# jczarnowski/DeepFactors

Hardware: NVIDIA H100
Metric: keyframe-pair Jacobian+JtJ evals/sec (640x480, C=32) (higher is better)
Workload: dtype f32

## Files before the change

### deepfactors_b200/csrc/dfk_api.cu

```cuda
#include <cuda_runtime.h>
#include <math.h>
#include <stdint.h>
#include <stdio.h>
#include <stdlib.h>
#include <string.h>

#include <algorithm>
#include <cmath>
#include <memory>
#include <new>
#include <string>
#include <vector>

#include "dfk.h"
#include "dfk_internal.h"

using namespace dfk;

namespace {

template <typename T, bool Pinned>
struct Scratch {
  T* ptr = nullptr;
  size_t cap = 0;

  Scratch() = default;
  Scratch(Scratch&& o) noexcept : ptr(o.ptr), cap(o.cap) { o.ptr = nullptr; o.cap = 0; }
  ~Scratch() { release(); }

  void release()
  {
    if constexpr (Pinned) cudaFreeHost(ptr);
    else cudaFree(ptr);
    ptr = nullptr;
    cap = 0;
  }
  cudaError_t ensure(size_t need)
  {
    if (cap >= need) return cudaSuccess;
    const size_t n = std::max(need, cap * 2);
    release();
    void* p = nullptr;
    const cudaError_t e = Pinned ? cudaMallocHost(&p, n * sizeof(T)) : cudaMalloc(&p, n * sizeof(T));
    if (e != cudaSuccess) return e;
    ptr = static_cast<T*>(p);
    cap = n;
    return e;
  }
};
template <typename T>
using DeviceBuf = Scratch<T, false>;
template <typename T>
using PinnedBuf = Scratch<T, true>;

}

struct DfkContext {
  int device = 0;
  int num_sms = 1;
  int sm_limit = 0;
  cudaStream_t own_stream = nullptr;
  cudaStream_t stream = nullptr;
  std::string err;
  DfkSfmAlignerParams params;
  DfkGramMode gram_mode = DFK_GRAM_AUTO;
  float se3_huber_delta = 0.1f;

  DeviceBuf<float> simple_scratch;
  DeviceBuf<unsigned int> counter;
  DeviceBuf<float> out_dev;
  PinnedBuf<float> out_host;
  DeviceBuf<float> code_dev;
  DeviceBuf<float> track_dev;
  PinnedBuf<float> track_host;
  DeviceBuf<unsigned char> batch_dev;
  PinnedBuf<unsigned char> batch_host;
  DeviceBuf<float> batch_partials;
  DeviceBuf<unsigned int> batch_counters;

  DeviceBuf<unsigned char> sparse_dev;
  PinnedBuf<unsigned char> sparse_host;
  DeviceBuf<unsigned char> rep_dev;
  std::vector<unsigned char> rep_host;
  DeviceBuf<unsigned char> geo_dev;
  std::vector<unsigned char> geo_host;
  DeviceBuf<SfmItemDev> items_dev;
  DeviceBuf<float> partials_dev;
  DeviceBuf<int> window_lists;
  DeviceBuf<int> marg_lists;
  DeviceBuf<double> marg_code;
  DeviceBuf<double> marg_dev;
  struct RayTab {
    float fx, fy, u0, v0;
    uint32_t w, h;
    DeviceBuf<float> dev;
    bool built;
  };
  std::vector<RayTab> ray_cache;
  std::vector<size_t> ray_pending;
  bool ray_flush = false;
  DeviceBuf<float> codes_dev;
  std::vector<float> codes_host;
  DeviceBuf<float> records_dev;
  PinnedBuf<float> records_host;
  std::vector<SfmItemDev> items_host;

  bool profiling = false;
  std::vector<cudaEvent_t> ev_pool;
  size_t ev_used = 0;
  double ev_ms_accum = 0.0;
  uint64_t ev_count_accum = 0;
  uint64_t launches = 0;

  ~DfkContext()
  {
    for (cudaEvent_t e : ev_pool) cudaEventDestroy(e);
    if (own_stream) cudaStreamDestroy(own_stream);
  }
};

struct DfkSfmStream {
  int device = 0, code_size = 0, max_items = 0, depth = 0;
  size_t max_bytes = 0;
  cudaStream_t copy_stream = nullptr;
  struct Slot {
    DeviceBuf<unsigned char> dev;
    DeviceBuf<float> rec_dev;
    PinnedBuf<float> rec_host;
    cudaEvent_t uploaded = nullptr, done = nullptr;
    int n = 0;
    uint64_t ticket = 0;
    bool busy = false;
  };
  std::vector<Slot> slots;
  std::vector<DfkSfmWorkItem> dev_items;
  uint64_t next_ticket = 0, next_wait = 0;
};

struct DfkWindow {
  int device = 0;
  WindowDev dev{};
  DeviceBuf<int> ints;
  DeviceBuf<float> areas;
  size_t floats = 0;
  std::vector<int> pair_k0, pair_k1, link_k0, link_k1, item_pair;
  std::vector<int> prior_ptr{0}, prior_kf, blk_i, blk_j;
  std::vector<long long> prior_off;
  DeviceBuf<int> kp_ints;
  DeviceBuf<long long> kp_off;
  KfPriorDev kp{};
};

struct DfkWindowSolver {
  int device = 0;
  int num_vars = 0, code_size = 0, num_keyframes = 0;
  WindowSolverDev* dev = nullptr;
  ~DfkWindowSolver() { window_solver_destroy(dev); }
};

namespace {

DfkStatus fail(DfkHandle h, DfkStatus s, const std::string& msg)
{
  if (h) h->err = msg;
  return s;
}

DfkStatus oom(DfkHandle h) noexcept
{
  if (h) {
    try {
      h->err = "out of host memory";
    } catch (...) {
    }
  }
  return DFK_ERR_NOMEM;
}

template <class F>
DfkStatus guarded(DfkHandle h, F&& body) noexcept
{
  if (!h) return DFK_ERR_INVALID_ARG;
  try {
    return body();
  } catch (...) {
    return oom(h);
  }
}
// ... 277 lines not shown
    if (fused) d.flags |= ITEM_FLAG_FUSED_DEPTH;
  }
  const int T = (int)tile_cursor;
  int G = std::min(max_ctas, T);
  if (G < 1) G = 1;
  plan->num_items = n;
  plan->num_tiles = T;
  plan->num_ctas = G;
  uint32_t partial_cursor = 0;
  int c = 0;
  for (int i = 0; i < n; ++i) {
    SfmItemDev& d = h->items_host[i];
    const long long tb = d.tile_begin, te = tb + d.num_tiles;
    while ((long long)(c + 1) * T / G <= tb) ++c;
    int first = c, last = c;
    while ((long long)(last + 1) * T / G < te) ++last;
    d.first_cta = (uint32_t)first;
    d.num_ctas = (uint32_t)(last - first + 1);
    d.partial_begin = partial_cursor;
    partial_cursor += d.num_ctas;
  }
  plan->num_partials = (int)partial_cursor;
  return DFK_OK;
}

constexpr size_t kMaxEventPairs = 8192;

DfkStatus drain_events(DfkHandle h)
{
  if (h->ev_used == 0) return DFK_OK;
  DFK_CUDA(h, cudaStreamSynchronize(h->stream), "profiling: stream synchronize failed");
  for (size_t k = 0; k < h->ev_used; ++k) {
    float ms = 0.f;
    DFK_CUDA(h, cudaEventElapsedTime(&ms, h->ev_pool[2 * k], h->ev_pool[2 * k + 1]), "profiling: event read failed");
    h->ev_ms_accum += ms;
  }
  h->ev_count_accum += h->ev_used;
  h->ev_used = 0;
  return DFK_OK;
}

DfkStatus profile_events(DfkHandle h, cudaEvent_t* e0, cudaEvent_t* e1)
{
  if (h->ev_used == kMaxEventPairs) DFK_TRY(drain_events(h));
  while (h->ev_pool.size() < 2 * (h->ev_used + 1)) {
    cudaEvent_t e;
    DFK_CUDA(h, cudaEventCreate(&e), "profiling: event creation failed");
    h->ev_pool.push_back(e);
  }
  *e0 = h->ev_pool[2 * h->ev_used];
  *e1 = h->ev_pool[2 * h->ev_used + 1];
  h->ev_used += 1;
  return DFK_OK;
}

DfkStatus run_batch(DfkHandle h, const DfkSfmWorkItem* items, int n, int code_size, float* records_dev)
{
  if (!items || n <= 0 || !records_dev) return fail(h, DFK_ERR_INVALID_ARG, "[SfmAligner::RunStep] null/empty batch");
  const bool wide = sfm_wide_supported(code_size);
  if (!sfm_fp32_supported(code_size) && !wide)
    return fail(h, DFK_ERR_UNSUPPORTED,
                "[SfmAligner::RunStep] no kernel instantiated for code size " + std::to_string(code_size));
  const bool tc_ok = sfm_tc_supported(code_size) || sfm_tc_wide_supported(code_size);
  bool tc = (h->gram_mode == DFK_GRAM_TF32X3) || (h->gram_mode == DFK_GRAM_AUTO && tc_ok);
  if (tc) {
    bool grads_ok = true;
    for (int i = 0; i < n && grads_ok; ++i)
      grads_ok = items[i].grad1.ptr && aligned(items[i].grad1.ptr, 8) && (items[i].grad1.pitch_bytes % 8 == 0);
    if (!grads_ok) {
      if (h->gram_mode == DFK_GRAM_TF32X3)
        return fail(h, DFK_ERR_UNSUPPORTED, "[SfmAligner::RunStep] tensor-core path needs 8-byte aligned grad1 rows");
      tc = false;
    }
  }
  if (tc && !tc_ok)
    return fail(h, DFK_ERR_UNSUPPORTED,
                "[SfmAligner::RunStep] tensor-core Gram path is not instantiated for code size " +
                    std::to_string(code_size));
  DeviceGuard guard(h->device);
  SfmLaunchPlan plan;
  const int tile_px = tc ? sfm_tc_tile_pixels(code_size) : (wide ? sfm_wide_tile_pixels(code_size) : kTilePixels);
  bool any_fused = false;
  for (int i = 0; i < n; ++i) any_fused = any_fused || items[i].code != nullptr;
  if (any_fused) {
    DFK_CUDA(h, h->codes_dev.ensure((size_t)n * code_size), "[SfmAligner::RunStep] scratch allocation failed");
    h->codes_host.assign((size_t)n * code_size, 0.0f);
  }
  const int ctas_per_sm = tc ? sfm_tc_ctas_per_sm(code_size) : (wide ? 1 : sfm_fp32_ctas_per_sm(code_size));
  const int sms = (h->sm_limit > 0 && h->sm_limit < h->num_sms) ? h->sm_limit : h->num_sms;
  DFK_TRY(build_items(h, items, n, code_size, tile_px, ctas_per_sm * sms, h->codes_dev.ptr, &plan));
  if (any_fused)
    DFK_CUDA(h, cudaMemcpyAsync(h->codes_dev.ptr, h->codes_host.data(), sizeof(float) * (size_t)n * code_size,
                                cudaMemcpyHostToDevice, h->stream),
             "[SfmAligner::RunStep] code upload failed");
  const size_t pfloats = tc ? sfm_tc_partial_floats(code_size) : sfm_partial_floats(code_size);
  DFK_CUDA(h, h->items_dev.ensure((size_t)n), "[SfmAligner::RunStep] scratch allocation failed");
  DFK_CUDA(h, h->partials_dev.ensure((size_t)plan.num_partials * pfloats), "[SfmAligner::RunStep] scratch allocation failed");
  SfmItemDev* items_dev = h->items_dev.ptr;
  float* partials_dev = h->partials_dev.ptr;
  DFK_CUDA(h, cudaMemcpyAsync(items_dev, h->items_host.data(), sizeof(SfmItemDev) * n, cudaMemcpyHostToDevice, h->stream),
           "[SfmAligner::RunStep] work list upload failed");
  if (!h->ray_pending.empty()) {
    DFK_CUDA(h, launch_sfm_ray_tables(items_dev, n, h->stream), "[SfmAligner::RunStep] kernel launch failed");
    for (size_t rt : h->ray_pending) h->ray_cache[rt].built = true;
    h->launches += 1;
  }
  cudaEvent_t ev0 = nullptr, ev1 = nullptr;
  if (h->profiling) DFK_TRY(profile_events(h, &ev0, &ev1));
  if (tc && wide) {
    DFK_CUDA(h, launch_sfm_tc_wide(code_size, items_dev, plan, partials_dev, h->stream, ev0, ev1),
             "[SfmAligner::RunStep] kernel launch failed");
  } else if (tc) {
    DFK_CUDA(h, launch_sfm_tc(items_dev, plan, partials_dev, h->stream, ev0, ev1),
             "[SfmAligner::RunStep] kernel launch failed");
  } else if (wide) {
    DFK_CUDA(h, launch_sfm_wide(code_size, items_dev, plan, partials_dev, h->stream, ev0, ev1),
             "[SfmAligner::RunStep] kernel launch failed");
  } else {
    DFK_CUDA(h, launch_sfm_fp32(code_size, items_dev, plan, partials_dev, h->stream, ev0, ev1),
             "[SfmAligner::RunStep] kernel launch failed");
  }
  DFK_CUDA(h, launch_sfm_finalize(code_size, tc, items_dev, n, partials_dev, records_dev, h->stream),
           "[SfmAligner::RunStep] kernel launch failed");
  h->launches += 2;
  return DFK_OK;
}

template <class Item>
struct Sparse;

template <>
struct Sparse<DfkReprojectionItem> {
  using Dev = ReprojItemDev;
  static constexpr int codes = 1;
  static constexpr size_t unit_bytes = 4 * sizeof(float);
  static constexpr const char* units = "matches";
  static size_t count(const DfkReprojectionItem& it) { return (size_t)it.num_matches; }
  static const char* error(const DfkReprojectionItem& it, int code_size)
  {
    if (!it.code || !it.query_xy || !it.train_xy) return "null argument";
    if (it.num_matches < 1 || !(it.sigma > 0.0f)) return "no matches / non-positive sigma";
    const uint32_t W = it.prx_orig.width, H = it.prx_orig.height;
    if (W == 0 || H == 0 || !img_ok(&it.prx_orig, W, H, 1) || !img_ok(&it.prx_jac, W, H, code_size))
      return "inconsistent image views";
    return nullptr;
  }
  static void pack(const DfkReprojectionItem& it, int code_size, size_t begin, size_t total, Dev& d, float* code,
                   const float* code_dev, unsigned char* payload)
  {
    d = Dev{{}, view_of(&it.prx_orig), view_of(&it.prx_jac), code_dev, (int)it.prx_orig.width, (int)it.prx_orig.height,
            it.num_matches, (int)begin, it.cauchy_delta, it.sigma};
    set_relative_pose(d.sp, it.pose1, it.pose0, it.cam);
    memcpy(code, it.code, sizeof(float) * code_size);
    float* query = reinterpret_cast<float*>(payload);
    memcpy(query + 2 * begin, it.query_xy, sizeof(float) * 2 * it.num_matches);
    memcpy(query + 2 * (total + begin), it.train_xy, sizeof(float) * 2 * it.num_matches);
  }
};

template <>
struct Sparse<DfkSparseGeometricItem> {
  using Dev = GeoItemDev;
  static constexpr int codes = 2;
  static constexpr size_t unit_bytes = 2 * sizeof(int32_t);
  static constexpr const char* units = "points";
  static size_t count(const DfkSparseGeometricItem& it) { return (size_t)it.num_points; }
  static const char* error(const DfkSparseGeometricItem& it, int code_size)
  {
    if (!it.code0 || !it.code1 || !it.points_xy) return "null argument";
    if (it.num_points < 1 || !(it.huber_delta > 0.0f)) return "no points / non-positive huber delta";
    const uint32_t W = it.prx0_orig.width, H = it.prx0_orig.height;
    if (W == 0 || H == 0 || !img_ok(&it.prx0_orig, W, H, 1) || !img_ok(&it.prx0_jac, W, H, code_size) ||
        !img_ok(&it.prx1_orig, W, H, 1) || !img_ok(&it.prx1_jac, W, H, code_size) || !img_ok(&it.dpt_grad1, W, H, 2))
      return "inconsistent image views";
    if (!cam_ok(&it.cam, W, H)) return "camera larger than the image views";
    return nullptr;
  }
  static void pack(const DfkSparseGeometricItem& it, int code_size, size_t begin, size_t , Dev& d, float* code,
                   const float* code_dev, unsigned char* payload)
  {
    d = Dev{{}, view_of(&it.prx0_orig), view_of(&it.prx0_jac), view_of(&it.prx1_orig), view_of(&it.prx1_jac),
            view_of(&it.dpt_grad1), code_dev, code_dev + code_size, it.cam.width, it.cam.height, (int)it.prx0_orig.width,
            (int)it.prx0_orig.height, it.num_points, (int)begin, it.huber_delta};
    set_relative_pose(d.sp, it.pose1, it.pose0, it.cam);
// ... 1379 lines not shown
```

### deepfactors_b200/csrc/dfk_internal.h

```cpp
#pragma once

#include <cuda_runtime.h>
#include <stdint.h>

#include <string>
#include <vector>

#include "dfk.h"

namespace dfk {

struct SfmItemDev {
  float q[4];
  float t[3];
  float R[9];
  float fx, fy, u0, v0;
  float border;
  float ulim;
  float vlim;
  float min_dpt, avg_dpt, huber_delta;
  const float* img0;
  const float* img1;
  const float* dpt0;
  float* valid0;
  const float* jac;
  const float* grad1;
  uint32_t img0_pitch, img1_pitch, dpt0_pitch, valid0_pitch, jac_pitch, grad1_pitch;
  uint32_t width, height;
  uint32_t num_pixels;
  uint32_t tile_begin;
  uint32_t num_tiles;
  uint32_t perm_mul;
  uint32_t mag_tiles;
  uint32_t mag_width;
  uint32_t first_cta, num_ctas, partial_begin;
  uint32_t flags;
  float* dpt_out;
  uint32_t dpt_out_pitch;
  const float* code;
  const float* ray_tab;
  float P0[36];
  float P1[36];
};

enum : uint32_t { ITEM_FLAG_BULK = 1u, ITEM_FLAG_GRAD_ALIGNED = 2u, ITEM_FLAG_FUSED_DEPTH = 4u };

template <int C>
struct SfmCfg {
  static constexpr int NF = C + 7;
  static constexpr int NFP = (NF + 7) & ~7;
  static constexpr int NB = NFP / 8;
  static constexpr int NBLK = NB * (NB + 1) / 2;
  static constexpr int PARTIAL_FLOATS = NFP * NFP + 8;
};

constexpr int kTilePixels = 256;

template <int C>
struct TcCfg {
  static constexpr int S = C - 8;
  static constexpr int F = C + 8;
  static constexpr int ROWS = 2 * C;
  static constexpr int COLS = C + 24;
  static constexpr int PARTIAL_FLOATS = ROWS * COLS + 8;
  static constexpr int INLIERS = ROWS * COLS;
  __host__ __device__ static constexpr int hh(int i, int j) { return j * ROWS + S + i; }
  __host__ __device__ static constexpr int lh(int i, int j) { return i < S ? j * ROWS + i : (16 + i) * ROWS + S + j; }
};

constexpr int sfm_tc_tile_pixels(int) { return 128; }
constexpr int sfm_tc_ctas_per_sm(int code_size) { return code_size <= 32 ? 4 : (code_size <= 64 ? 2 : 1); }
constexpr size_t sfm_tc_partial_floats(int code_size) { return (size_t)(2 * code_size) * (code_size + 24) + 8; }

constexpr int kTcTilePixels = sfm_tc_tile_pixels(32);
constexpr int kTcCtasPerSm = sfm_tc_ctas_per_sm(32);
constexpr int kTcRows = TcCfg<32>::ROWS;
constexpr int kTcCols = TcCfg<32>::COLS;
constexpr int kTcRowsPad = kTcRows;
constexpr int kTcPartialFloats = TcCfg<32>::PARTIAL_FLOATS;

struct SfmLaunchPlan {
  int num_items = 0;
  int num_tiles = 0;
  int num_ctas = 0;
  int num_partials = 0;
};

cudaError_t launch_sfm_fp32(int code_size, const SfmItemDev* items_dev, const SfmLaunchPlan& plan,
                            float* partials_dev, cudaStream_t stream, cudaEvent_t ev_start = nullptr,
                            cudaEvent_t ev_stop = nullptr);
cudaError_t launch_sfm_ray_tables(const SfmItemDev* items_dev, int num_items, cudaStream_t stream);
cudaError_t launch_sfm_finalize(int code_size, bool tc, const SfmItemDev* items_dev, int num_items,
                                const float* partials_dev, float* records_dev, cudaStream_t stream);
constexpr int sfm_wide_tile_pixels(int code_size) { return code_size >= 128 ? 64 : 128; }
bool sfm_wide_supported(int code_size);
cudaError_t launch_sfm_wide(int code_size, const SfmItemDev* items_dev, const SfmLaunchPlan& plan,
                            float* partials_dev, cudaStream_t stream, cudaEvent_t ev_start = nullptr,
                            cudaEvent_t ev_stop = nullptr);
bool sfm_tc_supported(int code_size);
cudaError_t launch_sfm_tc(const SfmItemDev* items_dev, const SfmLaunchPlan& plan, float* partials_dev,
                          cudaStream_t stream, cudaEvent_t ev_start = nullptr, cudaEvent_t ev_stop = nullptr);
bool sfm_tc_wide_supported(int code_size);
cudaError_t launch_sfm_tc_wide(int code_size, const SfmItemDev* items_dev, const SfmLaunchPlan& plan,
                               float* partials_dev, cudaStream_t stream, cudaEvent_t ev_start = nullptr,
                               cudaEvent_t ev_stop = nullptr);
size_t sfm_partial_floats(int code_size);
constexpr int sfm_fp32_ctas_per_sm(int code_size) { return code_size <= 8 ? 2 : 1; }
bool sfm_fp32_supported(int code_size);
int sfm_max_ctas();

struct PixelCam {
  float q[4], t[3];
  float fx, fy, u0, v0, border, ulim, vlim, min_dpt;
};
struct View {
  const float* ptr;
  uint32_t pitch;
};
cudaError_t launch_se3_step(const PixelCam& pc, float huber_delta, int width, int height, View img0, View img1,
                            View dpt0, View grad1, bool grad_aligned, float* scratch, unsigned int* counter,
                            float* out_dev , cudaStream_t s,
                            float* pose_dev = nullptr ,
                            float* history_dev = nullptr );
struct Se3TrackDesc {
  PixelCam pc;
  View img0, img1, dpt0, grad1;
  int width, height;
  int nblocks;
  int grad_aligned;
};
int se3_step_blocks(int width, int height);
cudaError_t launch_se3_track_batch(const Se3TrackDesc* descs_dev, int num_problems, int max_blocks, float huber_delta,
                                   float* scratch, int scratch_stride, unsigned int* counters, float* outs, float* poses,
                                   cudaStream_t s);
cudaError_t launch_eval_error(const PixelCam& pc, float huber_delta, int width, int height, View img0, View img1,
                              View dpt0, float* scratch, unsigned int* counter, float* out_dev , cudaStream_t s);
cudaError_t launch_warp(const PixelCam& pc, int width, int height, View img0, View img1, View dpt0, float* img2,
                        uint32_t img2_pitch, float* scratch, unsigned int* counter, float* out_dev ,
                        cudaStream_t s);
cudaError_t launch_update_depth(const float* code_dev, int code_size, int width, int height, View prx_orig, View jac,
                                float avg_dpt, float* dpt, uint32_t dpt_pitch, cudaStream_t s);
cudaError_t launch_sobel(int width, int height, View img, float* grad, uint32_t grad_pitch, cudaStream_t s);
cudaError_t launch_blur_down(int in_w, int in_h, View in, int out_w, int out_h, float* out, uint32_t out_pitch,
                             cudaStream_t s);
cudaError_t launch_squared_error(int width, int height, View a, View b, float* scratch, unsigned int* counter,
                                 float* out_dev, cudaStream_t s);
struct WindowDev {
  int num_keyframes, num_pairs, num_items, code_size;
  const int* kf0_ptr;
  const int* kf0_items;
  const int* kf1_ptr;
  const int* kf1_items;
  const int* pair_ptr;
  const int* pair_items;
  const float* item_area;
  int num_links;
  const int* lk0_ptr;
  const int* lk0_links;
  const int* lk1_ptr;
  const int* lk1_links;
  int num_frames;
  const int* frame_pair;
// ... 107 lines not shown
```

### deepfactors_b200/csrc/dfk_sfm_finalize.cu

```cuda
#include <cuda_runtime.h>
#include <stdint.h>

#include "dfk_internal.h"

namespace dfk {

namespace {

constexpr int kFinWarps = 8;
constexpr int kFinUnroll = 4;

__device__ __forceinline__ int packed_index(int i, int j, int NP) { return i * NP - (i * (i - 1)) / 2 + (j - i); }

template <int C, bool TC>
__global__ void __launch_bounds__(kFinWarps * 32)
sfm_finalize_kernel(const SfmItemDev* __restrict__ items, const float* __restrict__ partials,
                    float* __restrict__ records)
{
  using Cfg = SfmCfg<C>;
  constexpr int NFP = Cfg::NFP;
  constexpr int NP = 12 + C;
  constexpr int NH = NP * (NP + 1) / 2;
  constexpr int REC = NH + NP + 2;
  constexpr int NE = (C + 7 > 49) ? (C + 7) : 49;
  constexpr int EPL = (NE + 31) / 32;
  using Tc = TcCfg<C>;
  constexpr int PSTRIDE = TC ? Tc::PARTIAL_FLOATS : Cfg::PARTIAL_FLOATS;
  constexpr int INL_OFF = TC ? Tc::INLIERS : NFP * NFP;
  constexpr int NOFF = TC ? 3 : 1;
  __shared__ float red[kFinWarps][EPL * 32];
  __shared__ unsigned int red_inl[kFinWarps];
  __shared__ float sum[EPL * 32];

  cudaGridDependencySynchronize();
  const SfmItemDev& I = items[blockIdx.x];
  const int unit = blockIdx.y;
  const int warp = threadIdx.x >> 5, lane = threadIdx.x & 31;
  const float* P = partials + (size_t)I.partial_begin * PSTRIDE;
  const int np = (int)I.num_ctas;

  int off[EPL][NOFF];
  bool act[EPL];
#pragma unroll
  for (int q = 0; q < EPL; ++q) {
    const int e = q * 32 + lane;
    int fi, fj;
    if (unit < C) {
      act[q] = (unit + e) < (C + 7);
      fi = unit;
      fj = unit + e;
    } else {
      const int r = e / 7, c = e - 7 * r;
      act[q] = (e < 49) && (c >= r);
      fi = C + r;
      fj = C + c;
    }
    if (!act[q]) {
      fi = 0;
      fj = 0;
    }
    if constexpr (TC) {
      off[q][0] = Tc::hh(fi, fj);
      off[q][1] = Tc::lh(fi, fj);
      off[q][2] = Tc::lh(fj, fi);
    } else {
      off[q][0] = fi * NFP + fj;
    }
  }
  float part[EPL];
#pragma unroll
  for (int q = 0; q < EPL; ++q) part[q] = 0.0f;
  unsigned int inl = 0;
  for (int k0 = warp; k0 < np; k0 += kFinWarps * kFinUnroll) {
    float v[kFinUnroll][EPL];
    unsigned int vi[kFinUnroll];
#pragma unroll
    for (int u = 0; u < kFinUnroll; ++u) {
      const int k = k0 + u * kFinWarps;
      const bool on = k < np;
      const float* Pk = P + (size_t)(on ? k : 0) * PSTRIDE;
#pragma unroll
      for (int q = 0; q < EPL; ++q) {
        v[u][q] = 0.0f;
        if (on && act[q]) {
          if constexpr (TC) v[u][q] = (Pk[off[q][0]] + Pk[off[q][1]]) + Pk[off[q][2]];
          else v[u][q] = Pk[off[q][0]];
        }
      }
      vi[u] = (on && unit == C && lane == 0) ? reinterpret_cast<const unsigned int*>(Pk)[INL_OFF] : 0u;
    }
#pragma unroll
    for (int u = 0; u < kFinUnroll; ++u) {
#pragma unroll
      for (int q = 0; q < EPL; ++q) part[q] += v[u][q];
      inl += vi[u];
    }
  }
#pragma unroll
  for (int q = 0; q < EPL; ++q) red[warp][q * 32 + lane] = part[q];
  if (lane == 0) red_inl[warp] = inl;
  __syncthreads();
  if (warp == 0) {
#pragma unroll
    for (int q = 0; q < EPL; ++q) {
      float s = 0.0f;
#pragma unroll
      for (int w = 0; w < kFinWarps; ++w) s += red[w][q * 32 + lane];
      sum[q * 32 + lane] = s;
    }
  }
  __syncthreads();

  float* rec = records + (size_t)blockIdx.x * REC;
  float* JtJ = rec;
  float* Jtr = rec + NH;
  if (unit < C) {
    const int c = unit;
    for (int e = threadIdx.x; e < C - c; e += blockDim.x) JtJ[packed_index(12 + c, 12 + c + e, NP)] = sum[e];
    if (threadIdx.x < 12) {
      const int j = threadIdx.x % 6;
      const float* Pm = threadIdx.x < 6 ? I.P0 : I.P1;
      float s = 0.0f;
#pragma unroll
      for (int k = 0; k < 6; ++k) s = fmaf(Pm[k * 6 + j], sum[(C - c) + k], s);
      JtJ[packed_index(threadIdx.x, 12 + c, NP)] = s;
    }
    if (threadIdx.x == 12) Jtr[12 + c] = sum[(C - c) + 6];
  } else {
    __shared__ float Gaa[6][6];
    __shared__ float T0[6][6];
    __shared__ float T1[6][6];
    if (threadIdx.x < 36) {
      const int r = threadIdx.x / 6, c = threadIdx.x % 6;
      Gaa[r][c] = (c >= r) ? sum[r * 7 + c] : sum[c * 7 + r];
    }
    __syncthreads();
    if (threadIdx.x < 72) {
      const int m = threadIdx.x / 36, r = (threadIdx.x % 36) / 6, c = threadIdx.x % 6;
      const float* Pm = m ? I.P1 : I.P0;
      float s = 0.0f;
#pragma unroll
      for (int k = 0; k < 6; ++k) s = fmaf(Gaa[r][k], Pm[k * 6 + c], s);
      (m ? T1 : T0)[r][c] = s;
    }
    __syncthreads();
    for (int e = threadIdx.x; e < 144; e += blockDim.x) {
      const int i = e / 12, j = e % 12;
      if (j < i) continue;
      const float* Pa = (i < 6) ? I.P0 : I.P1;
      const float(*Tb)[6] = (j < 6) ? T0 : T1;
      const int ii = i % 6, jj = j % 6;
      float s = 0.0f;
#pragma unroll
      for (int k = 0; k < 6; ++k) s = fmaf(Pa[k * 6 + ii], Tb[k][jj], s);
      JtJ[packed_index(i, j, NP)] = s;
    }
    if (threadIdx.x >= 160 && threadIdx.x < 172) {
      const int i = threadIdx.x - 160;
      const float* Pa = (i < 6) ? I.P0 : I.P1;
      float s = 0.0f;
#pragma unroll
      for (int k = 0; k < 6; ++k) s = fmaf(Pa[k * 6 + (i % 6)], sum[k * 7 + 6], s);
      Jtr[i] = s;
    }
    if (threadIdx.x == 192) {
      unsigned int tot = 0;
      for (int w = 0; w < kFinWarps; ++w) tot += red_inl[w];
      rec[NH + NP] = sum[48];
      reinterpret_cast<unsigned int*>(rec)[NH + NP + 1] = tot;
    }
  }
}

template <int C, bool TC>
cudaError_t launch_fin(const SfmItemDev* items_dev, int num_items, const float* partials_dev, float* records_dev,
                       cudaStream_t stream)
{
  cudaLaunchConfig_t cfg{};
  cfg.gridDim = dim3(num_items, C + 1);
  cfg.blockDim = dim3(kFinWarps * 32);
  cfg.dynamicSmemBytes = 0;
  cfg.stream = stream;
  cudaLaunchAttribute attr[1];
  attr[0].id = cudaLaunchAttributeProgrammaticStreamSerialization;
  attr[0].val.programmaticStreamSerializationAllowed = 1;
  cfg.attrs = attr;
  cfg.numAttrs = 1;
  return cudaLaunchKernelEx(&cfg, sfm_finalize_kernel<C, TC>, items_dev, partials_dev, records_dev);
}

}

cudaError_t launch_sfm_finalize(int code_size, bool tc, const SfmItemDev* items_dev, int num_items,
                                const float* partials_dev, float* records_dev, cudaStream_t stream)
{
  if (tc) {
    switch (code_size) {
      case 32: return launch_fin<32, true>(items_dev, num_items, partials_dev, records_dev, stream);
      case 64: return launch_fin<64, true>(items_dev, num_items, partials_dev, records_dev, stream);
      case 128: return launch_fin<128, true>(items_dev, num_items, partials_dev, records_dev, stream);
      default: return cudaErrorInvalidValue;
    }
  }
  switch (code_size) {
    case 8: return launch_fin<8, false>(items_dev, num_items, partials_dev, records_dev, stream);
    case 16: return launch_fin<16, false>(items_dev, num_items, partials_dev, records_dev, stream);
    case 32: return launch_fin<32, false>(items_dev, num_items, partials_dev, records_dev, stream);
    case 64: return launch_fin<64, false>(items_dev, num_items, partials_dev, records_dev, stream);
    case 128: return launch_fin<128, false>(items_dev, num_items, partials_dev, records_dev, stream);
    default: return cudaErrorInvalidValue;
  }
}

}
```

### deepfactors_b200/csrc/dfk_sfm_tc.cu

```cuda
#include <cuda_runtime.h>
#include <stdint.h>
#include <stdio.h>
#include <stdlib.h>

#include "dfk_async.cuh"
#include "dfk_geom.cuh"
#include "dfk_internal.h"
#include "dfk_sfm_frontend.cuh"
#include "dfk_sfm_tc_common.cuh"
#include "dfk_wgmma.cuh"

namespace dfk {

namespace {

constexpr int C = 32;
constexpr int TILE = kTcTilePixels;
constexpr int THREADS = 128;
constexpr int NWARP = THREADS / 32;
constexpr uint32_t kLbo = 128 + 16;
constexpr uint32_t kSbo = 32 * kLbo + 16;
constexpr uint32_t OP_BYTES = 10 * kSbo;
#ifndef DFK_FLUSH_TILES
#define DFK_FLUSH_TILES 8
#endif
constexpr int kFlushTiles = DFK_FLUSH_TILES;

struct Smem {
  alignas(128) unsigned char op[OP_BYTES];
  SfmItem<C> item[NWARP];
};

__global__ void __launch_bounds__(THREADS, kTcCtasPerSm)
sfm_step_tc_kernel(const SfmItemDev* __restrict__ items, int num_tiles, float* __restrict__ partials)
{
  extern __shared__ __align__(128) unsigned char smem_raw[];
  Smem& sm = *reinterpret_cast<Smem*>(smem_raw);
  const int tid = threadIdx.x;
  const int warp = tid >> 5;
  const int lane = tid & 31;
  int g_lo, g_hi;
  cta_tiles(num_tiles, g_lo, g_hi);
  const int ntiles = g_hi - g_lo;
  if (ntiles <= 0) return;

  for (int e = tid; e < (int)(OP_BYTES / 16); e += THREADS)
    reinterpret_cast<float4*>(sm.op)[e] = make_float4(0.f, 0.f, 0.f, 0.f);
  __syncthreads();

  const uint32_t op = smem_u32(sm.op);
  const int c = lane & 7, r = lane >> 3;
  const uint32_t in_group = (uint32_t)(8 * warp) * kLbo + (uint32_t)(c & 1) * 64u + (uint32_t)r * 4u;
  const uint32_t code_l = op + (uint32_t)((c >> 1) < 3 ? (c >> 1) : 8) * kSbo + in_group;
  const uint32_t code_h = op + (uint32_t)(3 + (c >> 1)) * kSbo + in_group;
  const uint32_t pose_h = op + 7u * kSbo + (uint32_t)(8 * warp + (lane >> 2)) * kLbo + (uint32_t)(lane & 3) * 4u;
  const uint32_t pose_l = pose_h + 2u * kSbo;

  float acc[28];
#pragma unroll
  for (int q = 0; q < 28; ++q) acc[q] = 0.0f;
  SfmItem<C>& I = sm.item[warp];
  int it = 0;
  int cur_item = -1;
  uint32_t item_hi = 0;
  int tiles_in_chain = 0, chain_valid = 0, pslot = 0;
  bool fresh = true;
  unsigned int inliers = 0;

  auto flush = [&](bool item_end) {
    wgmma_wait_all();
    float* P = partials + (size_t)pslot * kTcPartialFloats;
    if (fresh || chain_valid > 0) {
      const int m0 = 16 * warp + (lane >> 2);
#pragma unroll
      for (int q = 0; q < 28; ++q) {
        const int m = m0 + 8 * ((q >> 1) & 1);
        const int n = 8 * (q >> 2) + 2 * (lane & 3) + (q & 1);
        if (n < 40 || m >= 24)
          put_partial(P + n * kTcRowsPad + m, chain_valid > 0 ? acc[q] : 0.0f, fresh);
      }
    }
    if (item_end && tid == 0) reinterpret_cast<unsigned int*>(P)[kTcRowsPad * kTcCols] = inliers;
    fresh = false;
    chain_valid = 0;
    tiles_in_chain = 0;
  };

  for (int i = 0; i < ntiles; ++i) {
    const int g = g_lo + i;
    if (cur_item < 0 || (uint32_t)g >= item_hi) {
      if (cur_item >= 0) flush(true);
      while ((uint32_t)g >= items[it].tile_begin + items[it].num_tiles) ++it;
      __syncwarp();
      load_item(I, items[it], lane, (int)blockIdx.x);
      load_code(I, items[it], C, lane, 32);
      __syncwarp();
      cur_item = it;
      item_hi = I.tile_begin + I.num_tiles;
      pslot = (int)I.slot;
      fresh = true;
      inliers = 0;
    } else if (tiles_in_chain == kFlushTiles) {
      flush(false);
    }
    uint32_t n;
    const uint32_t p0 = tile_origin<TILE>(I, g, n);
    const uint32_t s = 32u * (uint32_t)warp + (uint32_t)lane;
    const bool inb = s < n;
    const bool blk_live = 32u * (uint32_t)warp < n;
    const uint32_t W = I.width;
    const bool a16 = (I.flags & ITEM_FLAG_BULK) != 0;
    const bool fused = (I.flags & ITEM_FLAG_FUSED_DEPTH) != 0;
    uint32_t x0;
    const uint32_t y0 = div_magic(blk_live ? p0 + 32u * (uint32_t)warp : p0, W, I.mag_width, x0);
    uint32_t pxx = x0 + (inb ? (uint32_t)lane : 0u), py = y0;
    while (pxx >= W) {
      pxx -= W;
      ++py;
    }
    const float* __restrict__ jac = I.jac;
    const uint32_t joff = py * I.jac_pitch + pxx * C;
    float feat[8];
    bool ok = false;
    if (blk_live) {
      const float2 ray = table_ray(I, pxx, py);
      float d = ld_stream(I.dpt0 + (size_t)py * I.dpt0_pitch + pxx);
      const float i0 = ld_stream(I.img0 + (size_t)py * I.img0_pitch + pxx);
      if (fused) {
        const float4 cc = *reinterpret_cast<const float4*>(&I.code[4 * (lane & 7)]);
        float mine = 0.0f;
#pragma unroll
        for (int i8 = 0; i8 < 8; ++i8) {
          const uint32_t offk = __shfl_sync(0xffffffffu, joff, 4 * i8 + (lane >> 3));
          float p = chunk_dot(load_chunk_l1(jac + offk + 4 * (lane & 7), a16), cc);
          p = __fadd_rn(p, __shfl_xor_sync(0xffffffffu, p, 4));
          p = __fadd_rn(p, __shfl_xor_sync(0xffffffffu, p, 2));
          p = __fadd_rn(p, __shfl_xor_sync(0xffffffffu, p, 1));
          const float got = __shfl_sync(0xffffffffu, p, 8 * (lane & 3));
          if ((lane >> 2) == i8) mine = got;
        }
        d = prx_to_depth(__fadd_rn(d, mine), I.avg_dpt);
        if (inb) I.dpt_out[(size_t)py * I.dpt_out_pitch + pxx] = d;
      }
      if (inb) ok = pixel_row(I, pxx, py, ray, d, i0, true, feat);
    }
    if (!ok) {
#pragma unroll
      for (int f = 0; f < 8; ++f) feat[f] = 0.0f;
    }
    const unsigned bal = __ballot_sync(0xffffffffu, ok);
    float4 v[8];
#pragma unroll
    for (int i8 = 0; i8 < 8; ++i8) {
      const uint32_t offk = __shfl_sync(0xffffffffu, joff, 4 * i8 + r);
      v[i8] = make_float4(0.f, 0.f, 0.f, 0.f);
      if ((bal >> (4 * i8 + r)) & 1u) v[i8] = load_chunk(jac + offk + 4 * c, a16);
    }
    wgmma_wait_all();
#pragma unroll
    for (int i8 = 0; i8 < 8; ++i8) {
      const float sk = __shfl_sync(0xffffffffu, feat[0], 4 * i8 + r);
      const float x[4] = {sk * v[i8].x, sk * v[i8].y, sk * v[i8].z, sk * v[i8].w};
#pragma unroll
      for (int e = 0; e < 4; ++e) {
        const float h = tf32_trunc(x[e]);
// ... 53 lines not shown
```

### deepfactors_b200/csrc/dfk_window.cu

```cuda
#include <cuda_runtime.h>
#include <stdint.h>

#include "dfk_internal.h"

namespace dfk {

namespace {

__device__ __forceinline__ int packed_index(int i, int j, int NP) { return i * NP - (i * (i - 1)) / 2 + (j - i); }
__device__ __forceinline__ float rec_h(const float* rec, int a, int b, int NP)
{
  return a <= b ? rec[packed_index(a, b, NP)] : rec[packed_index(b, a, NP)];
}

__device__ __forceinline__ int link_row0(int r) { return r < 6 ? r : 6 + r; }
__device__ __forceinline__ int link_row1(int r, int C) { return r < 6 ? 6 + r : 6 + C + r; }

__global__ void __launch_bounds__(256)
window_assemble_kernel(WindowDev w, const float* __restrict__ records, const float* __restrict__ geo,
                       float* __restrict__ out)
{
  const int C = w.code_size, B = 6 + C, NP = 12 + C;
  const int NH = NP * (NP + 1) / 2, REC = NH + NP + 2;
  const int NG = 12 + 2 * C, NHG = NG * (NG + 1) / 2, RECG = NHG + NG + 2;
  float* tail = out + (size_t)w.num_keyframes * (B * B + B) + (size_t)w.num_pairs * B * 6;
  const int job = blockIdx.x;
  if (job < w.num_keyframes) {
    const int k = job;
    float* D = out + (size_t)k * B * B;
    float* g = out + (size_t)w.num_keyframes * B * B + (size_t)k * B;
    const int a0 = w.kf0_ptr[k], a1 = w.kf0_ptr[k + 1];
    const int b0 = w.kf1_ptr[k], b1 = w.kf1_ptr[k + 1];
    const int l00 = w.lk0_ptr[k], l01 = w.lk0_ptr[k + 1];
    const int l10 = w.lk1_ptr[k], l11 = w.lk1_ptr[k + 1];
    for (int e = threadIdx.x; e < B * B + B; e += blockDim.x) {
      float s = 0.0f;
      if (e < B * B) {
        const int r = e / B, c = e - r * B;
        const int lr = r < 6 ? r : 6 + r, lc = c < 6 ? c : 6 + c;
        for (int q = a0; q < a1; ++q) s += rec_h(records + (size_t)w.kf0_items[q] * REC, lr, lc, NP);
        if (r < 6 && c < 6)
          for (int q = b0; q < b1; ++q) s += rec_h(records + (size_t)w.kf1_items[q] * REC, 6 + r, 6 + c, NP);
        for (int q = l00; q < l01; ++q) s += rec_h(geo + (size_t)w.lk0_links[q] * RECG, link_row0(r), link_row0(c), NG);
        for (int q = l10; q < l11; ++q)
          s += rec_h(geo + (size_t)w.lk1_links[q] * RECG, link_row1(r, C), link_row1(c, C), NG);
        D[e] = s;
      } else {
        const int r = e - B * B;
        const int lr = r < 6 ? r : 6 + r;
        for (int q = a0; q < a1; ++q) s -= records[(size_t)w.kf0_items[q] * REC + NH + lr];
        if (r < 6)
          for (int q = b0; q < b1; ++q) s -= records[(size_t)w.kf1_items[q] * REC + NH + 6 + r];
        for (int q = l00; q < l01; ++q) s -= geo[(size_t)w.lk0_links[q] * RECG + NHG + link_row0(r)];
        for (int q = l10; q < l11; ++q) s -= geo[(size_t)w.lk1_links[q] * RECG + NHG + link_row1(r, C)];
        g[r] = s;
      }
    }
  } else if (job < w.num_keyframes + w.num_pairs) {
    const int p = job - w.num_keyframes;
    float* O = out + (size_t)w.num_keyframes * (B * B + B) + (size_t)p * B * 6;
    const int i0 = w.pair_ptr[p], i1 = w.pair_ptr[p + 1];
    for (int e = threadIdx.x; e < B * 6; e += blockDim.x) {
      const int r = e / 6, c = e - r * 6;
      const int lr = r < 6 ? r : 6 + r;
      float s = 0.0f;
      for (int q = i0; q < i1; ++q) s += rec_h(records + (size_t)w.pair_items[q] * REC, lr, 6 + c, NP);
      O[e] = s;
    }
  } else if (job < w.num_keyframes + w.num_pairs + w.num_links) {
    const int l = job - w.num_keyframes - w.num_pairs;
    float* O = tail + 2 + (size_t)l * B * B;
    const float* rec = geo + (size_t)l * RECG;
    for (int e = threadIdx.x; e < B * B; e += blockDim.x) {
      const int r = e / B, c = e - r * B;
      O[e] = rec_h(rec, link_row0(r), link_row1(c, C), NG);
    }
  } else if (job < w.num_keyframes + w.num_pairs + w.num_links + w.num_frames) {
    const int f = job - w.num_keyframes - w.num_pairs - w.num_links;
    float* Df = tail + 2 + (size_t)w.num_links * B * B + (size_t)f * 36;
    float* gf = tail + 2 + (size_t)w.num_links * B * B + (size_t)w.num_frames * 36 + (size_t)f * 6;
    const int p = w.frame_pair[f];
    const int i0 = w.pair_ptr[p], i1 = w.pair_ptr[p + 1];
    for (int e = threadIdx.x; e < 42; e += blockDim.x) {
      float s = 0.0f;
      if (e < 36) {
        const int r = e / 6, c = e - r * 6;
        for (int q = i0; q < i1; ++q) s += rec_h(records + (size_t)w.pair_items[q] * REC, 6 + r, 6 + c, NP);
        Df[e] = s;
      } else {
        for (int q = i0; q < i1; ++q) s -= records[(size_t)w.pair_items[q] * REC + NH + 6 + (e - 36)];
        gf[e - 36] = s;
      }
    }
  } else {
    __shared__ float red_f[8], red_i[8];
    float f = 0.0f, ni = 0.0f;
    for (int i = threadIdx.x; i < w.num_items; i += blockDim.x) {
      const float* rec = records + (size_t)i * REC;
      const uint32_t inl = __float_as_uint(rec[NH + NP + 1]);
      if (w.item_area[i] == 0.0f) {
        f += rec[NH + NP];
      } else {
        if (inl > 0) f += rec[NH + NP] / (float)inl * w.item_area[i];
        ni += (float)inl;
      }
    }
    for (int l = threadIdx.x; l < w.num_links; l += blockDim.x) f += geo[(size_t)l * RECG + NHG + NG];
    for (int o = 16; o > 0; o >>= 1) {
      f += __shfl_xor_sync(0xffffffffu, f, o);
// ... 343 lines not shown
          const double* d = md.kdelta + (size_t)kp.mem_ptr[f.idx] * B;
          double gd = 0.0;
          for (int c = 0; c < nB; ++c) gd = __fma_rn(P[(size_t)(a * B + r) * nB + c], d[c], gd);
          s += P[(size_t)nB * nB + a * B + r] - gd;
        }
      }
    }
    if (X == 0 && r >= 6 && md.w > 0.0) s -= md.w * md.code[r - 6];
    md.rhs[v] = s;
  }
  __shared__ double red[8];
  double f = 0.0;
  for (int q = 0; q < md.num_refs; ++q) {
    const KfMargRef fr = md.refs[q];
    if (fr.kind == 0) {
      if (threadIdx.x == 0) {
        const float* rec = md.records + (size_t)fr.idx * REC;
        const float area = w.item_area[fr.idx];
        const uint32_t inl = __float_as_uint(rec[NH + NP + 1]);
        if (area == 0.0f) f += (double)rec[NH + NP];
        else if (inl > 0) f += (double)rec[NH + NP] / (double)inl * (double)area;
      }
    } else if (fr.kind == 1) {
      if (threadIdx.x == 0) f += (double)md.geo[(size_t)fr.idx * RECG + NHG + NG];
    } else {
      const bool fp = fr.kind == 2;
      const int nB = fp ? B : (kp.mem_ptr[fr.idx + 1] - kp.mem_ptr[fr.idx]) * B;
      const double* P = fp ? md.fpriors + (size_t)fr.idx * PD : md.kpriors + kp.off[fr.idx];
      const double* d = fp ? md.fdelta + (size_t)fr.idx * B : md.kdelta + (size_t)kp.mem_ptr[fr.idx] * B;
      double gd = 0.0, dGd = 0.0;
      for (int r = threadIdx.x; r < nB; r += blockDim.x) {
        double Gd = 0.0;
        for (int c = 0; c < nB; ++c) Gd = __fma_rn(P[(size_t)r * nB + c], d[c], Gd);
        gd = __fma_rn(P[(size_t)nB * nB + r], d[r], gd);
        dGd = __fma_rn(d[r], Gd, dGd);
      }
      gd = block_sum(gd, red);
      dGd = block_sum(dGd, red);
      f = __dadd_rn(f, __dadd_rn(__fma_rn(-2.0, gd, P[(size_t)nB * nB + nB]), dGd));
    }
  }
  if (threadIdx.x == 0) {
    if (md.w > 0.0) {
      double cc = 0.0;
      for (int c = 0; c < C; ++c) cc = __fma_rn(md.code[c], md.code[c], cc);
      f = __fma_rn(md.w, cc, f);
    }
    *md.f = f;
    *md.info = 0;
  }
}

__global__ void __launch_bounds__(256)
window_marg_finalize_kernel(int C, KfMargDev md, int num_tiles, double* __restrict__ prior)
{
  const int B = 6 + C, n = md.n, nB = n * B;
  const bool bad = *md.info != 0;
  const int u = blockIdx.x, nt = n * (n + 1) / 2;
  if (u < nt) {
    const int t = n + 1 + u, I = md.tile_row[t], J = md.tile_col[t];
    const double* T = md.tiles + (size_t)t * B * B;
    for (int e = threadIdx.x; e < B * B; e += blockDim.x) {
      const int r = e / B, c = e - r * B;
      if (I == J && r < c) continue;
      const double v = bad ? 0.0 : T[e];
      prior[(size_t)((I - 1) * B + r) * nB + (J - 1) * B + c] = v;
      prior[(size_t)((J - 1) * B + c) * nB + (I - 1) * B + r] = v;
    }
    return;
  }
  for (int v = threadIdx.x; v < nB; v += blockDim.x) prior[(size_t)nB * nB + v] = bad ? 0.0 : md.rhs[B + v];
  if (threadIdx.x == 0) {
    double zz = 0.0;
    for (int r = 0; r < B; ++r) zz = __fma_rn(md.rhs[r], md.rhs[r], zz);
    prior[(size_t)nB * nB + nB] = bad ? 0.0 : __dsub_rn(*md.f, zz);
  }
}

}

cudaError_t launch_window_assemble(const WindowDev& w, const float* records_dev, const float* geo_records_dev,
                                   float* out_dev, cudaStream_t stream)
{
  window_assemble_kernel<<<w.num_keyframes + w.num_pairs + w.num_links + w.num_frames + 1, 256, 0, stream>>>(
      w, records_dev, geo_records_dev, out_dev);
  return cudaGetLastError();
}

cudaError_t launch_window_marginalize_frames(const WindowDev& w, const float* records_dev, int n, const int* frames_dev,
                                             double* priors_dev, int32_t* info_dev, cudaStream_t stream)
{
  window_marginalize_kernel<<<n, 256, 0, stream>>>(w, records_dev, frames_dev, priors_dev, info_dev);
  return cudaGetLastError();
}

cudaError_t launch_window_add_priors(const WindowDev& w, int m, const int* kf_ptr_dev, const int* kf_priors_dev,
                                     const double* priors_dev, const double* delta_dev, float* window_dev,
                                     cudaStream_t stream)
{
  window_add_priors_kernel<<<w.num_keyframes + 1, 256, 0, stream>>>(w, m, kf_ptr_dev, kf_priors_dev, priors_dev,
                                                                    delta_dev, window_dev);
  return cudaGetLastError();
}

cudaError_t launch_window_add_keyframe_priors(const WindowDev& w, const KfPriorDev& kp, const double* priors_dev,
                                              const double* delta_dev, float* window_dev, cudaStream_t stream)
{
  window_add_kf_priors_kernel<<<w.num_keyframes + kp.num_blocks + 1, 256, 0, stream>>>(w, kp, priors_dev, delta_dev,
                                                                                       window_dev);
  return cudaGetLastError();
}

cudaError_t launch_window_marg_gather(const WindowDev& w, const KfPriorDev& kp, const KfMargDev& md, int num_tiles,
                                      cudaStream_t stream)
{
  window_marg_gather_kernel<<<num_tiles + 1, 256, 0, stream>>>(w, kp, md, num_tiles);
  return cudaGetLastError();
}

cudaError_t launch_window_marg_finalize(int code_size, const KfMargDev& md, int num_tiles, double* prior_dev,
                                       cudaStream_t stream)
{
  window_marg_finalize_kernel<<<md.n * (md.n + 1) / 2 + 1, 256, 0, stream>>>(code_size, md, num_tiles, prior_dev);
  return cudaGetLastError();
}

}
```

Measured before the change: 32460.

## Compact TC partials to packed Gram, skip redundant uploads, enable PDL for assembly

Measured after the change: 34100, median of 6. 5.1% higher.

```diff
diff --git a/deepfactors_b200/csrc/dfk_api.cu b/deepfactors_b200/csrc/dfk_api.cu
--- a/deepfactors_b200/csrc/dfk_api.cu
+++ b/deepfactors_b200/csrc/dfk_api.cu
@@ -104,6 +104,9 @@
   DeviceBuf<float> records_dev;
   PinnedBuf<float> records_host;
   std::vector<SfmItemDev> items_host;
+  std::vector<SfmItemDev> items_sent;
+  std::vector<float> codes_sent;
+  cudaStream_t sent_stream = nullptr;
 
   bool profiling = false;
   std::vector<cudaEvent_t> ev_pool;
@@ -547,6 +550,7 @@
   const int tile_px = tc ? sfm_tc_tile_pixels(code_size) : (wide ? sfm_wide_tile_pixels(code_size) : kTilePixels);
   bool any_fused = false;
   for (int i = 0; i < n; ++i) any_fused = any_fused || items[i].code != nullptr;
+  const size_t items_cap = h->items_dev.cap, codes_cap = h->codes_dev.cap;
   if (any_fused) {
     DFK_CUDA(h, h->codes_dev.ensure((size_t)n * code_size), "[SfmAligner::RunStep] scratch allocation failed");
     h->codes_host.assign((size_t)n * code_size, 0.0f);
@@ -554,17 +558,28 @@
   const int ctas_per_sm = tc ? sfm_tc_ctas_per_sm(code_size) : (wide ? 1 : sfm_fp32_ctas_per_sm(code_size));
   const int sms = (h->sm_limit > 0 && h->sm_limit < h->num_sms) ? h->sm_limit : h->num_sms;
   DFK_TRY(build_items(h, items, n, code_size, tile_px, ctas_per_sm * sms, h->codes_dev.ptr, &plan));
-  if (any_fused)
-    DFK_CUDA(h, cudaMemcpyAsync(h->codes_dev.ptr, h->codes_host.data(), sizeof(float) * (size_t)n * code_size,
-                                cudaMemcpyHostToDevice, h->stream),
-             "[SfmAligner::RunStep] code upload failed");
   const size_t pfloats = tc ? sfm_tc_partial_floats(code_size) : sfm_partial_floats(code_size);
   DFK_CUDA(h, h->items_dev.ensure((size_t)n), "[SfmAligner::RunStep] scratch allocation failed");
   DFK_CUDA(h, h->partials_dev.ensure((size_t)plan.num_partials * pfloats), "[SfmAligner::RunStep] scratch allocation failed");
   SfmItemDev* items_dev = h->items_dev.ptr;
   float* partials_dev = h->partials_dev.ptr;
-  DFK_CUDA(h, cudaMemcpyAsync(items_dev, h->items_host.data(), sizeof(SfmItemDev) * n, cudaMemcpyHostToDevice, h->stream),
-           "[SfmAligner::RunStep] work list upload failed");
+  if (h->items_dev.cap != items_cap || h->codes_dev.cap != codes_cap) h->items_sent.clear();
+  const bool held = h->sent_stream == h->stream && h->items_sent.size() == (size_t)n &&
+                    memcmp(h->items_sent.data(), h->items_host.data(), sizeof(SfmItemDev) * n) == 0 &&
+                    (!any_fused || h->codes_sent == h->codes_host);
+  if (!held) {
+    h->items_sent.clear();
+    if (any_fused)
+      DFK_CUDA(h, cudaMemcpyAsync(h->codes_dev.ptr, h->codes_host.data(), sizeof(float) * (size_t)n * code_size,
+                                  cudaMemcpyHostToDevice, h->stream),
+               "[SfmAligner::RunStep] code upload failed");
+    DFK_CUDA(h, cudaMemcpyAsync(items_dev, h->items_host.data(), sizeof(SfmItemDev) * n, cudaMemcpyHostToDevice,
+                                h->stream),
+             "[SfmAligner::RunStep] work list upload failed");
+    h->items_sent = h->items_host;
+    if (any_fused) h->codes_sent = h->codes_host;
+    h->sent_stream = h->stream;
+  }
   if (!h->ray_pending.empty()) {
     DFK_CUDA(h, launch_sfm_ray_tables(items_dev, n, h->stream), "[SfmAligner::RunStep] kernel launch failed");
     for (size_t rt : h->ray_pending) h->ray_cache[rt].built = true;
diff --git a/deepfactors_b200/csrc/dfk_internal.h b/deepfactors_b200/csrc/dfk_internal.h
--- a/deepfactors_b200/csrc/dfk_internal.h
+++ b/deepfactors_b200/csrc/dfk_internal.h
@@ -64,20 +64,29 @@
   static constexpr int COLS = C + 24;
   static constexpr int PARTIAL_FLOATS = ROWS * COLS + 8;
   static constexpr int INLIERS = ROWS * COLS;
-  __host__ __device__ static constexpr int hh(int i, int j) { return j * ROWS + S + i; }
-  __host__ __device__ static constexpr int lh(int i, int j) { return i < S ? j * ROWS + i : (16 + i) * ROWS + S + j; }
+  __host__ __device__ static constexpr int hh(int i, int j, int ld = ROWS) { return j * ld + S + i; }
+  __host__ __device__ static constexpr int lh(int i, int j, int ld = ROWS) { return i < S ? j * ld + i : (16 + i) * ld + S + j; }
+};
+
+template <int C>
+struct TcGCfg {
+  static constexpr int NF = C + 7;
+  static constexpr int ENTRIES = NF * (NF + 1) / 2;
+  static constexpr int INLIERS = ENTRIES;
+  static constexpr int PARTIAL_FLOATS = (ENTRIES + 1 + 7) & ~7;
+  __host__ __device__ static constexpr int at(int i, int j) { return i * NF - (i * (i - 1)) / 2 + (j - i); }
 };
 
 constexpr int sfm_tc_tile_pixels(int) { return 128; }
 constexpr int sfm_tc_ctas_per_sm(int code_size) { return code_size <= 32 ? 4 : (code_size <= 64 ? 2 : 1); }
-constexpr size_t sfm_tc_partial_floats(int code_size) { return (size_t)(2 * code_size) * (code_size + 24) + 8; }
+constexpr size_t sfm_tc_partial_floats(int code_size)
+{
+  return code_size == 32 ? (size_t)TcGCfg<32>::PARTIAL_FLOATS : (size_t)(2 * code_size) * (code_size + 24) + 8;
+}
 
 constexpr int kTcTilePixels = sfm_tc_tile_pixels(32);
 constexpr int kTcCtasPerSm = sfm_tc_ctas_per_sm(32);
-constexpr int kTcRows = TcCfg<32>::ROWS;
-constexpr int kTcCols = TcCfg<32>::COLS;
-constexpr int kTcRowsPad = kTcRows;
-constexpr int kTcPartialFloats = TcCfg<32>::PARTIAL_FLOATS;
+constexpr int kTcPartialFloats = TcGCfg<32>::PARTIAL_FLOATS;
 
 struct SfmLaunchPlan {
   int num_items = 0;
diff --git a/deepfactors_b200/csrc/dfk_sfm_finalize.cu b/deepfactors_b200/csrc/dfk_sfm_finalize.cu
--- a/deepfactors_b200/csrc/dfk_sfm_finalize.cu
+++ b/deepfactors_b200/csrc/dfk_sfm_finalize.cu
@@ -10,9 +10,11 @@
 constexpr int kFinWarps = 8;
 constexpr int kFinUnroll = 4;
 
+enum PartFmt { PART_FP32, PART_TC_D, PART_TC_G };
+
 __device__ __forceinline__ int packed_index(int i, int j, int NP) { return i * NP - (i * (i - 1)) / 2 + (j - i); }
 
-template <int C, bool TC>
+template <int C, PartFmt FMT>
 __global__ void __launch_bounds__(kFinWarps * 32)
 sfm_finalize_kernel(const SfmItemDev* __restrict__ items, const float* __restrict__ partials,
                     float* __restrict__ records)
@@ -25,9 +27,11 @@
   constexpr int NE = (C + 7 > 49) ? (C + 7) : 49;
   constexpr int EPL = (NE + 31) / 32;
   using Tc = TcCfg<C>;
-  constexpr int PSTRIDE = TC ? Tc::PARTIAL_FLOATS : Cfg::PARTIAL_FLOATS;
-  constexpr int INL_OFF = TC ? Tc::INLIERS : NFP * NFP;
-  constexpr int NOFF = TC ? 3 : 1;
+  using Tg = TcGCfg<C>;
+  constexpr int PSTRIDE =
+      FMT == PART_TC_D ? Tc::PARTIAL_FLOATS : (FMT == PART_TC_G ? Tg::PARTIAL_FLOATS : Cfg::PARTIAL_FLOATS);
+  constexpr int INL_OFF = FMT == PART_TC_D ? Tc::INLIERS : (FMT == PART_TC_G ? Tg::INLIERS : NFP * NFP);
+  constexpr int NOFF = FMT == PART_TC_D ? 3 : 1;
   __shared__ float red[kFinWarps][EPL * 32];
   __shared__ unsigned int red_inl[kFinWarps];
   __shared__ float sum[EPL * 32];
@@ -59,10 +63,12 @@
       fi = 0;
       fj = 0;
     }
-    if constexpr (TC) {
+    if constexpr (FMT == PART_TC_D) {
       off[q][0] = Tc::hh(fi, fj);
       off[q][1] = Tc::lh(fi, fj);
       off[q][2] = Tc::lh(fj, fi);
+    } else if constexpr (FMT == PART_TC_G) {
+      off[q][0] = Tg::at(fi, fj);
     } else {
       off[q][0] = fi * NFP + fj;
     }
@@ -83,7 +89,7 @@
       for (int q = 0; q < EPL; ++q) {
         v[u][q] = 0.0f;
         if (on && act[q]) {
-          if constexpr (TC) v[u][q] = (Pk[off[q][0]] + Pk[off[q][1]]) + Pk[off[q][2]];
+          if constexpr (FMT == PART_TC_D) v[u][q] = (Pk[off[q][0]] + Pk[off[q][1]]) + Pk[off[q][2]];
           else v[u][q] = Pk[off[q][0]];
         }
       }
@@ -172,7 +178,7 @@
   }
 }
 
-template <int C, bool TC>
+template <int C, PartFmt FMT>
 cudaError_t launch_fin(const SfmItemDev* items_dev, int num_items, const float* partials_dev, float* records_dev,
                        cudaStream_t stream)
 {
@@ -186,7 +192,7 @@
   attr[0].val.programmaticStreamSerializationAllowed = 1;
   cfg.attrs = attr;
   cfg.numAttrs = 1;
-  return cudaLaunchKernelEx(&cfg, sfm_finalize_kernel<C, TC>, items_dev, partials_dev, records_dev);
+  return cudaLaunchKernelEx(&cfg, sfm_finalize_kernel<C, FMT>, items_dev, partials_dev, records_dev);
 }
 
 }
@@ -196,18 +202,18 @@
 {
   if (tc) {
     switch (code_size) {
-      case 32: return launch_fin<32, true>(items_dev, num_items, partials_dev, records_dev, stream);
-      case 64: return launch_fin<64, true>(items_dev, num_items, partials_dev, records_dev, stream);
-      case 128: return launch_fin<128, true>(items_dev, num_items, partials_dev, records_dev, stream);
+      case 32: return launch_fin<32, PART_TC_G>(items_dev, num_items, partials_dev, records_dev, stream);
+      case 64: return launch_fin<64, PART_TC_D>(items_dev, num_items, partials_dev, records_dev, stream);
+      case 128: return launch_fin<128, PART_TC_D>(items_dev, num_items, partials_dev, records_dev, stream);
       default: return cudaErrorInvalidValue;
     }
   }
   switch (code_size) {
-    case 8: return launch_fin<8, false>(items_dev, num_items, partials_dev, records_dev, stream);
-    case 16: return launch_fin<16, false>(items_dev, num_items, partials_dev, records_dev, stream);
-    case 32: return launch_fin<32, false>(items_dev, num_items, partials_dev, records_dev, stream);
-    case 64: return launch_fin<64, false>(items_dev, num_items, partials_dev, records_dev, stream);
-    case 128: return launch_fin<128, false>(items_dev, num_items, partials_dev, records_dev, stream);
+    case 8: return launch_fin<8, PART_FP32>(items_dev, num_items, partials_dev, records_dev, stream);
+    case 16: return launch_fin<16, PART_FP32>(items_dev, num_items, partials_dev, records_dev, stream);
+    case 32: return launch_fin<32, PART_FP32>(items_dev, num_items, partials_dev, records_dev, stream);
+    case 64: return launch_fin<64, PART_FP32>(items_dev, num_items, partials_dev, records_dev, stream);
+    case 128: return launch_fin<128, PART_FP32>(items_dev, num_items, partials_dev, records_dev, stream);
     default: return cudaErrorInvalidValue;
   }
 }
diff --git a/deepfactors_b200/csrc/dfk_sfm_tc.cu b/deepfactors_b200/csrc/dfk_sfm_tc.cu
--- a/deepfactors_b200/csrc/dfk_sfm_tc.cu
+++ b/deepfactors_b200/csrc/dfk_sfm_tc.cu
@@ -22,9 +22,14 @@
 constexpr uint32_t kSbo = 32 * kLbo + 16;
 constexpr uint32_t OP_BYTES = 10 * kSbo;
 #ifndef DFK_FLUSH_TILES
-#define DFK_FLUSH_TILES 8
+#define DFK_FLUSH_TILES 16
 #endif
 constexpr int kFlushTiles = DFK_FLUSH_TILES;
+using D = TcCfg<C>;
+using G = TcGCfg<C>;
+constexpr int kDsLd = D::COLS + 2;
+static_assert(D::ROWS * kDsLd * 4 <= 7 * kSbo, "staged D must fit into operand groups 0-6");
+__device__ __forceinline__ int staged(int o) { return (o % D::ROWS) * kDsLd + o / D::ROWS; }
 
 struct Smem {
   alignas(128) unsigned char op[OP_BYTES];
@@ -70,17 +75,28 @@
   auto flush = [&](bool item_end) {
     wgmma_wait_all();
     float* P = partials + (size_t)pslot * kTcPartialFloats;
-    if (fresh || chain_valid > 0) {
+    if (chain_valid > 0) {
+      float* Ds = reinterpret_cast<float*>(sm.op);
+      __syncthreads();
       const int m0 = 16 * warp + (lane >> 2);
 #pragma unroll
-      for (int q = 0; q < 28; ++q) {
+      for (int q = 0; q < 28; q += 2) {
         const int m = m0 + 8 * ((q >> 1) & 1);
-        const int n = 8 * (q >> 2) + 2 * (lane & 3) + (q & 1);
-        if (n < 40 || m >= 24)
-          put_partial(P + n * kTcRowsPad + m, chain_valid > 0 ? acc[q] : 0.0f, fresh);
-      }
-    }
-    if (item_end && tid == 0) reinterpret_cast<unsigned int*>(P)[kTcRowsPad * kTcCols] = inliers;
+        const int n = 8 * (q >> 2) + 2 * (lane & 3);
+        *reinterpret_cast<float2*>(Ds + m * kDsLd + n) = make_float2(acc[q], acc[q + 1]);
+      }
+      __syncthreads();
+      int i = 0, row = 0;
+      for (int e = tid; e < G::ENTRIES; e += THREADS) {
+        while (e - row >= G::NF - i) row += G::NF - i++;
+        const int j = i + (e - row);
+        put_partial(P + e, (Ds[staged(D::hh(i, j))] + Ds[staged(D::lh(i, j))]) + Ds[staged(D::lh(j, i))], fresh);
+      }
+      __syncthreads();
+    } else if (fresh) {
+      for (int e = tid; e < G::ENTRIES; e += THREADS) put_partial(P + e, 0.0f, true);
+    }
+    if (item_end && tid == 0) reinterpret_cast<unsigned int*>(P)[G::INLIERS] = inliers;
     fresh = false;
     chain_valid = 0;
     tiles_in_chain = 0;
diff --git a/deepfactors_b200/csrc/dfk_window.cu b/deepfactors_b200/csrc/dfk_window.cu
--- a/deepfactors_b200/csrc/dfk_window.cu
+++ b/deepfactors_b200/csrc/dfk_window.cu
@@ -25,6 +25,7 @@
   const int NG = 12 + 2 * C, NHG = NG * (NG + 1) / 2, RECG = NHG + NG + 2;
   float* tail = out + (size_t)w.num_keyframes * (B * B + B) + (size_t)w.num_pairs * B * 6;
   const int job = blockIdx.x;
+  cudaGridDependencySynchronize();
   if (job < w.num_keyframes) {
     const int k = job;
     float* D = out + (size_t)k * B * B;
@@ -534,9 +535,17 @@
 cudaError_t launch_window_assemble(const WindowDev& w, const float* records_dev, const float* geo_records_dev,
                                    float* out_dev, cudaStream_t stream)
 {
-  window_assemble_kernel<<<w.num_keyframes + w.num_pairs + w.num_links + w.num_frames + 1, 256, 0, stream>>>(
-      w, records_dev, geo_records_dev, out_dev);
-  return cudaGetLastError();
+  cudaLaunchConfig_t cfg{};
+  cfg.gridDim = dim3(w.num_keyframes + w.num_pairs + w.num_links + w.num_frames + 1);
+  cfg.blockDim = dim3(256);
+  cfg.dynamicSmemBytes = 0;
+  cfg.stream = stream;
+  cudaLaunchAttribute attr[1];
+  attr[0].id = cudaLaunchAttributeProgrammaticStreamSerialization;
+  attr[0].val.programmaticStreamSerializationAllowed = 1;
+  cfg.attrs = attr;
+  cfg.numAttrs = 1;
+  return cudaLaunchKernelEx(&cfg, window_assemble_kernel, w, records_dev, geo_records_dev, out_dev);
 }
 
 cudaError_t launch_window_marginalize_frames(const WindowDev& w, const float* records_dev, int n, const int* frames_dev,
```
